# deepinv/deepinv

Measured on NVIDIA H100. Metric: pnp_pgd_iterations_per_s, higher is better.
Workload: dtype f32 (3 x FP16 split-operand tensor-core GEMMs: 22-bit operands, fp32 accumulate) + f32 operators

## Files before the change

### deepinv_b200/csrc/conv_tc32.cu

```cuda
#include "common.cuh"
#ifndef DINVK_EMUL
#include "tc_ptx.cuh"
#include "tma_tile.cuh"
#include <cuda_fp16.h>
#else
namespace dinvk { namespace tc {
inline void ldg256(const void* p, uint32_t (&r)[8]) { std::memcpy(r, p, 32); }
inline void stg256(void* p, const uint32_t (&r)[8]) { std::memcpy(p, r, 32); }
} }
#endif

#include <algorithm>
#include <cstdlib>
#include <cstring>

namespace dinvk {
namespace t32 {

constexpr int TX = 16, TY = 8;
constexpr int A_TILE = 128 * 128;
constexpr int B_TILE = 128 * 128;
constexpr int STAGE = 2 * A_TILE + B_TILE;
constexpr int STAGES = 4;
constexpr int STG_WARP = 16 * 32;
constexpr int SMEM = STAGES * STAGE + 8 * STG_WARP * 4 + 1024;
constexpr int THREADS = 2 * 128 + 32;

__device__ __forceinline__ float rna_tf32(float x) {
#ifndef DINVK_EMUL
  uint32_t u;
  asm("cvt.rna.tf32.f32 %0, %1;" : "=r"(u) : "f"(x));
  return __uint_as_float(u);
#else
  return __uint_as_float((__float_as_uint(x) + 0x1000u) & 0xffffe000u);
#endif
}

struct FmtTF32 {
  using elem = float;
  static constexpr int CH = 16, EB = 4, ID = 0;
  static constexpr float CORR = 1.0f;
#ifndef DINVK_EMUL
  static constexpr CUtensorMapDataType TM = CU_TENSOR_MAP_DATA_TYPE_FLOAT32;
#endif
};
struct FmtF16 {
  using elem = __half;
  static constexpr int CH = 32, EB = 2, ID = 1;
  static constexpr float CORR = 4.8828125e-4f;
#ifndef DINVK_EMUL
  static constexpr CUtensorMapDataType TM = CU_TENSOR_MAP_DATA_TYPE_FLOAT16;
#endif
};

#ifndef DINVK_EMUL
template <class F>
__device__ __forceinline__ void mma(float* d, uint32_t a_lo, uint32_t a_hi, uint32_t b_lo, uint32_t b_hi, uint32_t accumulate) {
  if constexpr (F::ID == 0) tc::wgmma_tf32_n64(d, a_lo, a_hi, b_lo, b_hi, accumulate);
  else tc::wgmma_f16_n64(d, a_lo, a_hi, b_lo, b_hi, accumulate);
}
template <class F>
__device__ __forceinline__ void mma_block64(float* acc, uint32_t a, uint32_t a_hi, uint32_t b, uint32_t b_hi, uint32_t fresh) {
  mma<F>(acc, a, a_hi, b, b_hi, fresh);
  mma<F>(acc + 32, a, a_hi, b + 512, b_hi, fresh);
  mma<F>(acc, a + 2, a_hi, b + 2, b_hi, 1u);
  mma<F>(acc + 32, a + 2, a_hi, b + 514, b_hi, 1u);
  mma<F>(acc + 32, a + 4, a_hi, b, b_hi, 1u);
  mma<F>(acc + 32, a + 6, a_hi, b + 2, b_hi, 1u);
}
template <class F>
__device__ __forceinline__ void mma128(float* d, uint32_t a_lo, uint32_t a_hi, uint32_t b_lo, uint32_t b_hi, uint32_t accumulate) {
  if constexpr (F::ID == 0) tc::wgmma_tf32_n128(d, a_lo, a_hi, b_lo, b_hi, accumulate);
  else tc::wgmma_f16_n128(d, a_lo, a_hi, b_lo, b_hi, accumulate);
}
template <class F>
__device__ __forceinline__ void mma_block128(float* acc, uint32_t w, uint32_t w_hi, uint32_t x, uint32_t x_hi, uint32_t fresh) {
  mma128<F>(acc, w, w_hi, x, x_hi, fresh);
  mma128<F>(acc + 64, w + 512, w_hi, x, x_hi, fresh);
  mma128<F>(acc, w + 2, w_hi, x + 2, x_hi, 1u);
  mma128<F>(acc + 64, w + 514, w_hi, x + 2, x_hi, 1u);
  mma128<F>(acc + 64, w, w_hi, x + 4, x_hi, 1u);
  mma128<F>(acc + 64, w + 2, w_hi, x + 6, x_hi, 1u);
}
template <class F, int N>
__device__ __forceinline__ void drain(float* v, const float* acc) {
#pragma unroll
  for (int i = 0; i < N / 2; ++i) v[i] += acc[i] + acc[N / 2 + i] * F::CORR;
}

__device__ __forceinline__ void release_stage(uint64_t* bar) {
  __syncwarp();
  if ((threadIdx.x & 31) == 0) tc::mbar_arrive(bar);
}

struct Maps {
  CUtensorMap a[4];
  CUtensorMap b;
};

struct Params {
  int B, H, W, Cin, Cout;
  int ntaps, kc_per_tap;
  int dx[9], dy[9], amap[9];
  int mode;
  int tiles_x, tiles_y, n_tiles;
  int relu;
  int win;
  const void* res;
  const void* res2;
  void* out;
  int* flag;
  const float* bias;
  int ngrp;
};

__device__ __forceinline__ void tile_index(const Params& P, int pixel_tiles, int t, int& pt, int& nt) {
  const int u = t / P.ngrp, lo = t - u * P.ngrp;
  const int hi = u / pixel_tiles;
  pt = u - hi * pixel_tiles;
  nt = hi * P.ngrp + lo;
}

#endif
template <class F>
__device__ __forceinline__ bool store_split(typename F::elem* p, const float* v) {
  uint32_t u[4][8];
  bool bad = false;
  if constexpr (F::ID == 0) {
#pragma unroll
    for (int i = 0; i < 16; ++i) {
      const float hi = rna_tf32(v[i]);
      u[i >> 3][i & 7] = __float_as_uint(hi);
      u[2 + (i >> 3)][i & 7] = __float_as_uint(v[i] - hi);
    }
  } else {
#pragma unroll
    for (int i = 0; i < 32; i += 2) {
      const __half h0 = __float2half_rn(v[i]), h1 = __float2half_rn(v[i + 1]);
      const __half l0 = __float2half_rn((v[i] - __half2float(h0)) * 2048.0f), l1 = __float2half_rn((v[i + 1] - __half2float(h1)) * 2048.0f);
      bad |= !(fabsf(v[i]) < 65000.0f) || !(fabsf(v[i + 1]) < 65000.0f);
      u[i >> 4][(i >> 1) & 7] = (uint32_t)__half_as_ushort(h0) | ((uint32_t)__half_as_ushort(h1) << 16);
      u[2 + (i >> 4)][(i >> 1) & 7] = (uint32_t)__half_as_ushort(l0) | ((uint32_t)__half_as_ushort(l1) << 16);
    }
  }
  char* pc = reinterpret_cast<char*>(p);
#pragma unroll
  for (int k = 0; k < 4; ++k) tc::stg256(pc + 32 * k, u[k]);
  return bad;
}
template <class F>
__device__ __forceinline__ void add_split_raw(const uint32_t (*raw)[8], float* v) {
  if constexpr (F::ID == 0) {
#pragma unroll
    for (int e = 0; e < 8; ++e) {
      v[e] += __uint_as_float(raw[0][e]) + __uint_as_float(raw[2][e]);
      v[8 + e] += __uint_as_float(raw[1][e]) + __uint_as_float(raw[3][e]);
    }
  } else {
#pragma unroll
    for (int c = 0; c < 2; ++c)
#pragma unroll
      for (int e = 0; e < 8; ++e) {
        const float2 h = __half22float2(*reinterpret_cast<const __half2*>(&raw[c][e]));
        const float2 l = __half22float2(*reinterpret_cast<const __half2*>(&raw[2 + c][e]));
        v[c * 16 + 2 * e] += h.x + l.x * F::CORR;
        v[c * 16 + 2 * e + 1] += h.y + l.y * F::CORR;
      }
  }
}
template <class F>
__device__ __forceinline__ void add_split(const typename F::elem* p, float* v) {
  uint32_t raw[4][8];
  const char* pc = reinterpret_cast<const char*>(p);
#pragma unroll
  for (int k = 0; k < 4; ++k) tc::ldg256(pc + 32 * k, raw[k]);
  add_split_raw<F>(raw, v);
}

#ifndef DINVK_EMUL
template <class F>
// ... 167 lines not shown
  __shared__ __align__(8) uint64_t full_bar[STAGES];
  __shared__ __align__(8) uint64_t empty_bar[STAGES];

  const int warp = threadIdx.x >> 5, lane = threadIdx.x & 31;
  const int pixel_tiles = P.B * P.tiles_y * P.tiles_x;
  const int total_tiles = pixel_tiles * P.n_tiles;
  const int nk = P.ntaps * P.kc_per_tap;

  if (threadIdx.x == 0) {
    tc::prefetch_tmap(&M.a[0]);
    tc::prefetch_tmap(&M.b);
    for (int s = 0; s < STAGES; ++s) { tc::mbar_init(&full_bar[s], 1); tc::mbar_init(&empty_bar[s], 8); }
    tc::fence_barrier_init();
  }
  __syncthreads();

  if (warp == 8) {
    if (lane == 0) {
      int s = 0; uint32_t ph = 0;
      for (int t = blockIdx.x; t < total_tiles; t += gridDim.x) {
        int pt, nt; tile_index(P, pixel_tiles, t, pt, nt);
        const int b = pt / (P.tiles_y * P.tiles_x), r = pt - b * (P.tiles_y * P.tiles_x);
        const int y0 = (r / P.tiles_x) * TY, x0 = (r % P.tiles_x) * TX;
        for (int kb = 0; kb < nk; ++kb) {
          const int tap = kb / P.kc_per_tap, kc = kb - tap * P.kc_per_tap;
          tc::mbar_wait(&empty_bar[s], ph ^ 1);
          uint8_t* sa = smem + s * STAGE;
          tc::mbar_arrive_expect_tx(&full_bar[s], STAGE);
          tc::tma_load_4d(sa, &M.a[P.amap[tap]], &full_bar[s], (2 * kc) * (2 * F::CH), x0 + P.dx[tap], y0 + P.dy[tap], b);
          tc::tma_load_4d(sa + A_TILE, &M.a[P.amap[tap]], &full_bar[s], (2 * kc + 1) * (2 * F::CH), x0 + P.dx[tap], y0 + P.dy[tap], b);
          tc::tma_load_2d(sa + 2 * A_TILE, &M.b, &full_bar[s], tap * P.Cin + kc * (2 * F::CH), nt * 128);
          if (++s == STAGES) { s = 0; ph ^= 1; }
        }
      }
    }
  } else {
    const int wg = warp >> 2;
    constexpr uint32_t HI = tc::desc_hi_sw128(1024);
    const uint32_t smem_lo = tc::smem_u32(smem) >> 4;
    int s = 0; uint32_t ph = 0;
    for (int t = blockIdx.x; t < total_tiles; t += gridDim.x) {
      int pt, nt; tile_index(P, pixel_tiles, t, pt, nt);
      const int b = pt / (P.tiles_y * P.tiles_x), r = pt - b * (P.tiles_y * P.tiles_x);
      const int y0 = (r / P.tiles_x) * TY, x0 = (r % P.tiles_x) * TX;
      float acc[64], v[32];
#pragma unroll
      for (int i = 0; i < 64; ++i) acc[i] = 0.f;
#pragma unroll
      for (int i = 0; i < 32; ++i) v[i] = 0.f;
      int in_win = 0;
      for (int kb = 0; kb < nk; ++kb) {
        tc::mbar_wait(&full_bar[s], ph);
        const uint32_t a0 = smem_lo + static_cast<uint32_t>(s) * (STAGE >> 4) + static_cast<uint32_t>(wg * (64 * 128 >> 4));
        const uint32_t b0 = smem_lo + static_cast<uint32_t>(s) * (STAGE >> 4) + (2 * A_TILE >> 4);
        tc::wgmma_fence();
#pragma unroll
        for (int jj = 0; jj < 2; ++jj)
          mma_block64<F>(acc, a0 + jj * (A_TILE >> 4), HI, b0 + jj * 4, HI, (jj | in_win) != 0 ? 1u : 0u);
        tc::wgmma_commit();
        tc::wgmma_wait<0>();
        tc::reg_fence<64>(acc);
        release_stage(&empty_bar[s]);
        if (++in_win == P.win || kb == nk - 1) {
          drain<F, 64>(v, acc);
          in_win = 0;
        }
        if (++s == STAGES) { s = 0; ph ^= 1; }
      }
      const int tap = P.mode == 2 ? nt * 64 / P.Cout : 0;
      const auto pixel_of = [&](int m) -> long long {
        const int mm = 64 * wg + 16 * (warp & 3) + m;
        const int y = y0 + mm / TX, x = x0 + mm % TX;
        if (!(y < P.H && x < P.W)) return -1;
        if (P.mode == 2) return ((long long)b * (2 * P.H) + 2 * y + (tap >> 1)) * (2LL * P.W) + 2 * x + (tap & 1);
        return ((long long)b * P.H + y) * P.W + x;
      };
      epilogue<F>(P, v, reinterpret_cast<float*>(smem + STAGES * STAGE) + warp * STG_WARP, pixel_of, nt * 64 - tap * P.Cout);
    }
  }
}

namespace slab {
constexpr int TXP = 16, TYP = 16;
constexpr int SLAB_X = TXP + 8, SLAB_Y = TYP + 2;
constexpr int SLAB_BYTES = SLAB_X * SLAB_Y * 128;
constexpr int A_STAGES = 2, B_STAGES = 6;
constexpr int WT_TILE = 128 * 128;
constexpr int CONSUMER_WARPS = 8;
constexpr int SMEM_BYTES = A_STAGES * SLAB_BYTES + B_STAGES * WT_TILE + CONSUMER_WARPS * STG_WARP * 4 + 1024;
constexpr int THREADS = 32 * CONSUMER_WARPS + 128;
constexpr int PRODUCER_REGS = 40, CONSUMER_REGS = 232;
static_assert(SLAB_BYTES % 1024 == 0, "slab stages must stay 1024-byte aligned");
static_assert(SMEM_BYTES <= 227 * 1024, "shared memory budget");
}

template <class F>
__global__ void __launch_bounds__(slab::THREADS, 1) conv_tc32_slab_kernel(const __grid_constant__ Maps M, const Params P) {
  using namespace slab;
  extern __shared__ uint8_t smem_raw[];
  uint8_t* smem = reinterpret_cast<uint8_t*>((reinterpret_cast<uintptr_t>(smem_raw) + 1023) & ~static_cast<uintptr_t>(1023));
  uint8_t* smem_b = smem + A_STAGES * SLAB_BYTES;
  __shared__ __align__(8) uint64_t afull[A_STAGES];
  __shared__ __align__(8) uint64_t aempty[A_STAGES];
  __shared__ __align__(8) uint64_t bfull[B_STAGES];
  __shared__ __align__(8) uint64_t bempty[B_STAGES];

  const int warp = threadIdx.x >> 5, lane = threadIdx.x & 31;
  const int pixel_tiles = P.B * P.tiles_y * P.tiles_x;
  const int total_tiles = pixel_tiles * P.n_tiles;
  const int nblk = P.Cin / F::CH;

  if (threadIdx.x == 0) {
    tc::prefetch_tmap(&M.a[0]);
    tc::prefetch_tmap(&M.b);
    for (int s = 0; s < A_STAGES; ++s) { tc::mbar_init(&afull[s], 1); tc::mbar_init(&aempty[s], CONSUMER_WARPS); }
    for (int s = 0; s < B_STAGES; ++s) { tc::mbar_init(&bfull[s], 1); tc::mbar_init(&bempty[s], CONSUMER_WARPS); }
    tc::fence_barrier_init();
  }
  __syncthreads();

  if (warp >= CONSUMER_WARPS) {
    tc::setmaxnreg_dec<PRODUCER_REGS>();
    if (warp == CONSUMER_WARPS && lane == 0) {
      int sa = 0; uint32_t pha = 0;
      int sb = 0; uint32_t phb = 0;
      for (int t = blockIdx.x; t < total_tiles; t += gridDim.x) {
        int pt, nt; tile_index(P, pixel_tiles, t, pt, nt);
        const int b = pt / (P.tiles_y * P.tiles_x), r = pt - b * (P.tiles_y * P.tiles_x);
        const int y0 = (r / P.tiles_x) * TYP, x0 = (r % P.tiles_x) * TXP;
        for (int j = 0; j < nblk; ++j) {
          tc::mbar_wait(&aempty[sa], pha ^ 1);
          tc::mbar_arrive_expect_tx(&afull[sa], SLAB_BYTES);
          tc::tma_load_4d(smem + sa * SLAB_BYTES, &M.a[0], &afull[sa], j * (2 * F::CH), x0 - 1, y0 - 1, b);
          if (++sa == A_STAGES) { sa = 0; pha ^= 1; }
          for (int tp = 0; tp < 5; ++tp) {
            tc::mbar_wait(&bempty[sb], phb ^ 1);
            tc::mbar_arrive_expect_tx(&bfull[sb], WT_TILE);
            tc::tma_load_2d(smem_b + sb * WT_TILE, &M.b, &bfull[sb], (j * 5 + tp) * (2 * F::CH), nt * 128);
            if (++sb == B_STAGES) { sb = 0; phb ^= 1; }
          }
        }
      }
    }
  } else {
    tc::setmaxnreg_inc<CONSUMER_REGS>();
    const int wg = warp >> 2;
    constexpr uint32_t HI_X = tc::desc_hi_sw128(SLAB_X * 128);
    constexpr uint32_t HI_W = tc::desc_hi_sw128(1024);
    const uint32_t slab_lo0 = (tc::smem_u32(smem) >> 4) + static_cast<uint32_t>(wg * 8 * 8);
    const uint32_t bt_lo0 = tc::smem_u32(smem_b) >> 4;
    int sa = 0; uint32_t pha = 0;
    int sb = 0; uint32_t phb = 0;
    for (int t = blockIdx.x; t < total_tiles; t += gridDim.x) {
      int pt, nt; tile_index(P, pixel_tiles, t, pt, nt);
      const int b = pt / (P.tiles_y * P.tiles_x), r = pt - b * (P.tiles_y * P.tiles_x);
      const int y0 = (r / P.tiles_x) * TYP, x0 = (r % P.tiles_x) * TXP;
      float acc[128], v[64];
#pragma unroll
      for (int i = 0; i < 128; ++i) acc[i] = 0.f;
#pragma unroll
      for (int i = 0; i < 64; ++i) v[i] = 0.f;
      int in_win = 0;
      int pend_b = -1;
      for (int j = 0; j < nblk; ++j) {
        tc::mbar_wait(&afull[sa], pha);
        const uint32_t slab_lo = slab_lo0 + static_cast<uint32_t>(sa) * (SLAB_BYTES >> 4);
        const uint32_t fresh = in_win == 0 ? 0u : 1u;
        const bool last_of_win = (in_win + 1 == P.win) || (j == nblk - 1);
#pragma unroll
        for (int tp = 0; tp < 5; ++tp) {
          tc::mbar_wait(&bfull[sb], phb);
          const uint32_t b_lo = bt_lo0 + static_cast<uint32_t>(sb) * (WT_TILE >> 4);
          tc::wgmma_fence();
#pragma unroll
          for (int par = 0; par < 2; ++par) {
            const int tap = 2 * tp + par;
            if (tap < 9) {
              const uint32_t x_t = slab_lo + static_cast<uint32_t>((tap / 3) * SLAB_X + (tap % 3)) * 8;
              mma_block128<F>(acc, b_lo + par * 4, HI_W, x_t, HI_X, tap == 0 ? fresh : 1u);
            }
          }
          tc::wgmma_commit();
          if (tp == 4) {
            tc::wgmma_wait<0>();
            tc::reg_fence<128>(acc);
            if (pend_b >= 0) release_stage(&bempty[pend_b]);
            release_stage(&bempty[sb]);
            release_stage(&aempty[sa]);
            pend_b = -1;
            if (last_of_win) drain<F, 128>(v, acc);
          } else {
            tc::wgmma_wait<1>();
            if (pend_b >= 0) release_stage(&bempty[pend_b]);
            pend_b = sb;
          }
          if (++sb == B_STAGES) { sb = 0; phb ^= 1; }
        }
        if (++sa == A_STAGES) { sa = 0; pha ^= 1; }
        in_win = last_of_win ? 0 : in_win + 1;
      }
      const auto pixel_of = [&](int n) -> long long {
        const int y = y0 + (n >> 3), x = x0 + 8 * wg + (n & 7);
        return y < P.H && x < P.W ? ((long long)b * P.H + y) * P.W + x : -1;
      };
      epilogue_t<F>(P, v, reinterpret_cast<float*>(smem_b + B_STAGES * WT_TILE) + warp * STG_WARP, pixel_of, nt * 64 + 16 * (warp & 3));
    }
  }
}

#endif
struct HeadParams {
  const float* x; const float* w; const float* bias; void* out;
  int B, C, H, W, Cout;
  float fill_scalar; const float* fill_batch; int has_fill; int relu;
  int* flag;
};

template <class F, int CT>
__global__ void __launch_bounds__(256) head_tc32_kernel(const HeadParams P) {
  constexpr int KR = 9 * CT, KP = (KR + 3) & ~3;
#ifndef DINVK_EMUL
  extern __shared__ __align__(16) float sw[];
#else
  float* sw = reinterpret_cast<float*>(::emul::dyn_smem());
#endif
  for (int i = threadIdx.x; i < P.Cout * KP; i += blockDim.x) {
    const int co = i / KP, k = i - co * KP;
    sw[i] = k < KR ? __ldg(P.w + co * KR + k) : 0.f;
  }
  __syncthreads();
  const long long npix = (long long)P.B * P.H * P.W;
  const long long p = (long long)blockIdx.x * blockDim.x + threadIdx.x;
  if (p >= npix) return;
  const long long HW = (long long)P.H * P.W;
  const int b = (int)(p / HW);
  const int rem = (int)(p - (long long)b * HW);
  const int y = rem / P.W, x = rem - y * P.W;
  const float fillv = P.has_fill ? (P.fill_batch ? __ldg(P.fill_batch + b) : P.fill_scalar) : 0.f;
  float in[KP];
#pragma unroll
  for (int k = KR; k < KP; ++k) in[k] = 0.f;
  const float* img = P.x + (long long)b * P.C * HW;
#pragma unroll
  for (int c = 0; c < CT; ++c) {
#pragma unroll
    for (int tap = 0; tap < 9; ++tap) {
      const int yy = y + tap / 3 - 1, xx = x + tap % 3 - 1;
      const bool inb = (yy >= 0) && (yy < P.H) && (xx >= 0) && (xx < P.W);
      float val = 0.f;
      if (inb) val = (c < P.C) ? __ldg(img + (long long)c * HW + (long long)yy * P.W + xx) : fillv;
      in[c * 9 + tap] = val;
    }
  }
  typename F::elem* o = static_cast<typename F::elem*>(P.out) + p * P.Cout * 2;
  bool bad = false;
  for (int c0 = 0; c0 < P.Cout; c0 += F::CH) {
    float v[F::CH];
#pragma unroll
    for (int i = 0; i < F::CH; ++i) {
      float a = P.bias ? __ldg(P.bias + c0 + i) : 0.f;
      const float4* wr = reinterpret_cast<const float4*>(sw + (c0 + i) * KP);
#pragma unroll
      for (int k = 0; k < KP / 4; ++k) {
// ... 375 lines not shown
}

static int default_window() {
  static int w = -1;
  if (w < 0) {
    const char* e = getenv("DINVK_TC32_WINDOW");
    w = e ? std::max(1, atoi(e)) : 4;
  }
  return w;
}

template <class F>
static int conv_generic(const void* x, const void* weight, const float* bias, const void* res, const void* res2, void* out, int B, int H,
                        int W, int Cin, int Cout, int kind, int act, int window, int* flag, void* stream) {
  DINVK_CHECK_ARG(x && weight && out, "conv_tc32: null pointer");
  DINVK_CHECK_ARG(B >= 0 && H >= 1 && W >= 1, "conv_tc32: bad shape");
  DINVK_CHECK_ARG(kind >= 0 && kind <= 2, "conv_tc32: kind=%d not in 0..2", kind);
  DINVK_CHECK_ARG(Cin % (2 * F::CH) == 0 && Cin >= 2 * F::CH, "conv_tc32: Cin=%d must be a multiple of %d", Cin, 2 * F::CH);
  DINVK_CHECK_ARG(Cout % 64 == 0 && Cout >= 64, "conv_tc32: Cout=%d must be a multiple of 64", Cout);
  DINVK_CHECK_ARG(kind != 1 || (H % 2 == 0 && W % 2 == 0), "conv_tc32: 2x2 stride-2 needs even H, W");
  DINVK_CHECK_ARG(kind == 0 || (!res && !res2), "conv_tc32: residual inputs are for kind 0 only");
  DINVK_CHECK_ARG(epilogue_aligned(bias, res, res2, out), "conv_tc32: bias, res, res2 and out must be 16-byte aligned");
  if (B == 0) return DINVK_OK;
  Maps M;
  Params P{};
  int rc;
  const uint64_t px = (uint64_t)Cin * 2 * F::EB;
  P.B = B; P.Cin = Cin; P.Cout = Cout;
  P.kc_per_tap = Cin / (2 * F::CH);
  P.relu = act; P.res = res; P.res2 = res2; P.out = out; P.bias = bias; P.flag = flag;
  P.win = window > 0 ? window : default_window();
  const uint32_t abox[4] = {2 * F::CH, TX, TY, 1};
  long long K = Cin, rows = 2LL * Cout;
  if (kind == 1) {
    const int Ho = H / 2, Wo = W / 2;
    const uint64_t adims[4] = {(uint64_t)Cin * 2, (uint64_t)Wo, (uint64_t)Ho, (uint64_t)B}, astrides[3] = {2 * px, 2 * px * W, px * W * H};
    for (int t = 0; t < 4; ++t) {
      const char* base = reinterpret_cast<const char*>(x) + ((long long)(t >> 1) * W + (t & 1)) * px;
      if ((rc = map_split<F>(&M.a[t], base, 4, adims, astrides, abox, "tc32 activations"))) return rc;
      P.amap[t] = t;
    }
    K = 4LL * Cin;
    P.H = Ho; P.W = Wo; P.ntaps = 4; P.n_tiles = Cout / 64;
  } else {
    const uint64_t adims[4] = {(uint64_t)Cin * 2, (uint64_t)W, (uint64_t)H, (uint64_t)B}, astrides[3] = {px, px * W, px * W * H};
    if ((rc = map_split<F>(&M.a[0], x, 4, adims, astrides, abox, "tc32 activations"))) return rc;
    M.a[1] = M.a[0]; M.a[2] = M.a[0]; M.a[3] = M.a[0];
    P.H = H; P.W = W;
    if (kind == 0) {
      K = 9LL * Cin;
      P.ntaps = 9; P.n_tiles = Cout / 64;
      for (int t = 0; t < 9; ++t) { P.dx[t] = t % 3 - 1; P.dy[t] = t / 3 - 1; }
    } else {
      rows = 8LL * Cout;
      P.ntaps = 1; P.mode = 2; P.n_tiles = 4 * Cout / 64;
    }
  }
  const uint64_t wdims[2] = {(uint64_t)K, (uint64_t)rows}, wstride = (uint64_t)K * F::EB;
  const uint32_t wbox[2] = {2 * F::CH, 128};
  if ((rc = map_split<F>(&M.b, weight, 2, wdims, &wstride, wbox, "tc32 weights"))) return rc;
  P.tiles_x = ceil_div(P.W, TX); P.tiles_y = ceil_div(P.H, TY);
  P.ngrp = getenv("DINVK_TC32_NT_OUTER") ? 1 : P.n_tiles;
  return launch_persistent(conv_tc32_kernel<F>, THREADS, SMEM, (long long)P.B * P.tiles_y * P.tiles_x * P.n_tiles, stream, M, P);
}

template <class F>
static int conv_slab(const void* x, const void* weight, const float* bias, const void* res, const void* res2, void* out, int B, int H, int W,
                     int Cin, int Cout, int act, int window, int* flag, void* stream) {
  DINVK_CHECK_ARG(x && weight && out, "conv_tc32_slab: null pointer");
  DINVK_CHECK_ARG(B >= 0 && H >= 1 && W >= 1, "conv_tc32_slab: bad shape");
  DINVK_CHECK_ARG(Cin % F::CH == 0 && Cin >= F::CH, "conv_tc32_slab: Cin=%d must be a multiple of %d", Cin, F::CH);
  DINVK_CHECK_ARG(Cout % 64 == 0 && Cout >= 64, "conv_tc32_slab: Cout=%d must be a multiple of 64", Cout);
  DINVK_CHECK_ARG(epilogue_aligned(bias, res, res2, out), "conv_tc32_slab: bias, res, res2 and out must be 16-byte aligned");
  if (B == 0) return DINVK_OK;
  Maps M;
  Params P{};
  int rc;
  const uint64_t px = (uint64_t)Cin * 2 * F::EB;
  const uint64_t adims[4] = {(uint64_t)Cin * 2, (uint64_t)W, (uint64_t)H, (uint64_t)B}, astrides[3] = {px, px * W, px * W * H};
  const uint32_t abox[4] = {2 * F::CH, slab::SLAB_X, slab::SLAB_Y, 1};
  if ((rc = map_split<F>(&M.a[0], x, 4, adims, astrides, abox, "tc32 activations"))) return rc;
  M.a[1] = M.a[0]; M.a[2] = M.a[0]; M.a[3] = M.a[0];
  const uint64_t wdims[2] = {10ull * Cin, 2ull * Cout}, wstride = 10ull * Cin * F::EB;
  const uint32_t wbox[2] = {2 * F::CH, 128};
  if ((rc = map_split<F>(&M.b, weight, 2, wdims, &wstride, wbox, "tc32 weights"))) return rc;
  P.B = B; P.H = H; P.W = W; P.Cin = Cin; P.Cout = Cout;
  P.ntaps = 9; P.kc_per_tap = Cin / F::CH; P.n_tiles = Cout / 64;
  for (int t = 0; t < 9; ++t) { P.dx[t] = t % 3 - 1; P.dy[t] = t / 3 - 1; }
  P.relu = act; P.res = res; P.res2 = res2; P.out = out; P.bias = bias; P.flag = flag;
  static const int def_win = getenv("DINVK_TC32_SLAB_WINDOW") ? std::max(1, atoi(getenv("DINVK_TC32_SLAB_WINDOW"))) : 1;
  P.win = window > 0 ? window : def_win;
  P.tiles_x = ceil_div(W, slab::TXP); P.tiles_y = ceil_div(H, slab::TYP);
  {
    static const int env_g = getenv("DINVK_TC32_NT_GROUP") ? atoi(getenv("DINVK_TC32_NT_GROUP")) : 0;
    int g = env_g > 0 ? env_g : 2;
    while (g > 1 && P.n_tiles % g) --g;
    P.ngrp = std::max(1, std::min(g, P.n_tiles));
  }
  return launch_persistent(conv_tc32_slab_kernel<F>, slab::THREADS, slab::SMEM_BYTES, (long long)P.B * P.tiles_y * P.tiles_x * P.n_tiles,
                           stream, M, P);
}

#endif
template <class F>
static int conv_head(const float* x_nchw, const float* weight, const float* bias, void* out, int B, int C, int H, int W, int Cout,
                     float fill_scalar, const float* fill_batch, int has_fill, int act, int* flag, void* stream) {
  const int CT = C + (has_fill ? 1 : 0);
  DINVK_CHECK_ARG(Cout % F::CH == 0 && Cout >= F::CH && Cout <= 256, "conv_tc32_head: Cout=%d must be a multiple of %d (<= 256)", Cout, F::CH);
  HeadParams P{x_nchw, weight, bias, out, B, C, H, W, Cout, fill_scalar, fill_batch, has_fill, act, flag};
  const long long npix = (long long)B * H * W;
  static const bool old_head = getenv("DINVK_TC32_OLD_HEAD") != nullptr;
  if (Cout == 64 && CT >= 1 && CT <= 4 && !old_head) {
    const long long warps = (long long)B * ceil_div(H, 2) * ceil_div(W, 32);
    const unsigned g = (unsigned)((warps + 7) / 8);
    switch (CT) {
      case 1: DINVK_LAUNCH((head64_tc32_kernel<F, 1>), dim3(g), dim3(256), 0, stream, P); break;
      case 2: DINVK_LAUNCH((head64_tc32_kernel<F, 2>), dim3(g), dim3(256), 0, stream, P); break;
      case 3: DINVK_LAUNCH((head64_tc32_kernel<F, 3>), dim3(g), dim3(256), 0, stream, P); break;
      default: DINVK_LAUNCH((head64_tc32_kernel<F, 4>), dim3(g), dim3(256), 0, stream, P); break;
    }
    return DINVK_POST_LAUNCH();
  }
  const unsigned grid = (unsigned)((npix + 255) / 256);
  const size_t smem = (size_t)Cout * ((9 * CT + 3) & ~3) * 4;
  switch (CT) {
    case 1: DINVK_LAUNCH((head_tc32_kernel<F, 1>), dim3(grid), dim3(256), smem, stream, P); break;
    case 2: DINVK_LAUNCH((head_tc32_kernel<F, 2>), dim3(grid), dim3(256), smem, stream, P); break;
    case 3: DINVK_LAUNCH((head_tc32_kernel<F, 3>), dim3(grid), dim3(256), smem, stream, P); break;
    default: DINVK_LAUNCH((head_tc32_kernel<F, 4>), dim3(grid), dim3(256), smem, stream, P); break;
  }
  return DINVK_POST_LAUNCH();
}

template <class F>
static int conv_tail(const void* x, const float* weight, const float* bias, const float* add_nchw, float* out_nchw, int B, int H, int W,
                     int Cin, int Cout, const int* flag, void* stream) {
  DINVK_CHECK_ARG(Cin % F::CH == 0 && Cin >= F::CH && Cin <= 128, "conv_tc32_tail: Cin=%d must be a multiple of %d (<= 128)", Cin, F::CH);
  TailParams P{x, weight, bias, add_nchw, out_nchw, B, H, W, Cin, Cout, flag};
  static const bool old_tail = getenv("DINVK_TC32_OLD_TAIL") != nullptr;
  if (Cin == 64 && Cout >= 1 && Cout <= 4 && !old_tail) {
    const int co = Cout == 3 ? 4 : Cout, wt = 16 / co;
    const long long warps = (long long)B * ceil_div(W, wt) * ceil_div(H, TL_RC);
    const unsigned grid = (unsigned)((warps + 7) / 8);
    if (co == 1) DINVK_LAUNCH((tail64_tc32_kernel<F, 1>), dim3(grid), dim3(256), 0, stream, P);
    else if (co == 2) DINVK_LAUNCH((tail64_tc32_kernel<F, 2>), dim3(grid), dim3(256), 0, stream, P);
    else DINVK_LAUNCH((tail64_tc32_kernel<F, 4>), dim3(grid), dim3(256), 0, stream, P);
    return DINVK_POST_LAUNCH();
  }
  const int tiles = B * ceil_div(H, TL_TY) * ceil_div(W, TL_TX);
  const int CO = Cout <= 2 ? 2 : 4;
  const size_t smem = ((size_t)(TL_TY + 2) * (TL_TX + 2) * (Cin + 4) + (size_t)CO * 9 * Cin) * 4;
  int rc;
  if (CO == 2) {
    if ((rc = allow_smem(tail_tc32_kernel<F, 2>, smem))) return rc;
    DINVK_LAUNCH((tail_tc32_kernel<F, 2>), dim3(tiles), dim3(256), smem, stream, P);
  } else {
    if ((rc = allow_smem(tail_tc32_kernel<F, 4>, smem))) return rc;
    DINVK_LAUNCH((tail_tc32_kernel<F, 4>), dim3(tiles), dim3(256), smem, stream, P);
  }
  return DINVK_POST_LAUNCH();
}

}
}

using namespace dinvk;

#define DINVK_FMT_DISPATCH(fmt, call_tf32, call_f16)                                                   \
// ... 68 lines not shown
```

### deepinv_b200/csrc/tc_ptx.cuh

```cuda
#pragma once
#include <cstdint>
#include <cuda.h>
#include <cuda_bf16.h>
#include <cuda_runtime.h>

namespace dinvk {
namespace tc {

__device__ __forceinline__ uint32_t smem_u32(const void* p) { return static_cast<uint32_t>(__cvta_generic_to_shared(p)); }

__device__ __forceinline__ bool elect_one() {
  uint32_t pred = 0;
  asm volatile(
      "{\n\t"
      ".reg .pred P;\n\t"
      "elect.sync _|P, 0xffffffff;\n\t"
      "selp.u32 %0, 1, 0, P;\n\t"
      "}\n"
      : "=r"(pred));
  return pred != 0;
}

__device__ __forceinline__ void mbar_init(uint64_t* bar, uint32_t count) {
  asm volatile("mbarrier.init.shared::cta.b64 [%0], %1;" ::"r"(smem_u32(bar)), "r"(count));
}
__device__ __forceinline__ void fence_barrier_init() { asm volatile("fence.mbarrier_init.release.cluster;" ::: "memory"); }
__device__ __forceinline__ void fence_proxy_async() { asm volatile("fence.proxy.async.shared::cta;" ::: "memory"); }
__device__ __forceinline__ void mbar_arrive_expect_tx(uint64_t* bar, uint32_t bytes) {
  asm volatile("mbarrier.arrive.expect_tx.shared::cta.b64 _, [%0], %1;" ::"r"(smem_u32(bar)), "r"(bytes) : "memory");
}
__device__ __forceinline__ void mbar_arrive(uint64_t* bar) {
  asm volatile("mbarrier.arrive.shared::cta.b64 _, [%0];" ::"r"(smem_u32(bar)) : "memory");
}
__device__ __forceinline__ bool mbar_try_wait(uint64_t* bar, uint32_t parity) {
  uint32_t ok;
  asm volatile(
      "{\n\t"
      ".reg .pred P;\n\t"
      "mbarrier.try_wait.parity.shared::cta.b64 P, [%1], %2;\n\t"
      "selp.u32 %0, 1, 0, P;\n\t"
      "}\n"
      : "=r"(ok)
      : "r"(smem_u32(bar)), "r"(parity)
      : "memory");
  return ok != 0;
}
__device__ __forceinline__ void mbar_wait(uint64_t* bar, uint32_t parity) {
  while (!mbar_try_wait(bar, parity)) {
  }
}

__device__ __forceinline__ void prefetch_tmap(const CUtensorMap* m) {
  asm volatile("prefetch.tensormap [%0];" ::"l"(reinterpret_cast<uint64_t>(m)) : "memory");
}
__device__ __forceinline__ void tma_load_2d(void* smem, const CUtensorMap* m, uint64_t* bar, int c0, int c1) {
  asm volatile("cp.async.bulk.tensor.2d.shared::cluster.global.mbarrier::complete_tx::bytes [%0], [%1, {%3, %4}], [%2];" ::"r"(
                   smem_u32(smem)),
               "l"(reinterpret_cast<uint64_t>(m)), "r"(smem_u32(bar)), "r"(c0), "r"(c1)
               : "memory");
}
__device__ __forceinline__ void tma_load_4d(void* smem, const CUtensorMap* m, uint64_t* bar, int c0, int c1, int c2, int c3) {
  asm volatile(
      "cp.async.bulk.tensor.4d.shared::cluster.global.mbarrier::complete_tx::bytes [%0], [%1, {%3, %4, %5, %6}], [%2];" ::"r"(
          smem_u32(smem)),
      "l"(reinterpret_cast<uint64_t>(m)), "r"(smem_u32(bar)), "r"(c0), "r"(c1), "r"(c2), "r"(c3)
      : "memory");
}

__device__ __forceinline__ void wgmma_fence() { asm volatile("wgmma.fence.sync.aligned;" ::: "memory"); }
__device__ __forceinline__ void wgmma_commit() { asm volatile("wgmma.commit_group.sync.aligned;" ::: "memory"); }
template <int N>
__device__ __forceinline__ void wgmma_wait() { asm volatile("wgmma.wait_group.sync.aligned %0;" ::"n"(N) : "memory"); }
template <int N>
__device__ __forceinline__ void reg_fence(float* d) {
#pragma unroll
  for (int i = 0; i < N; ++i) asm volatile("" : "+f"(d[i])::"memory");
}

template <uint32_t N>
__device__ __forceinline__ void setmaxnreg_dec() { asm volatile("setmaxnreg.dec.sync.aligned.u32 %0;" ::"n"(N)); }
template <uint32_t N>
__device__ __forceinline__ void setmaxnreg_inc() { asm volatile("setmaxnreg.inc.sync.aligned.u32 %0;" ::"n"(N)); }

__host__ __device__ constexpr uint32_t desc_hi_sw128(uint32_t sbo_bytes) { return ((sbo_bytes >> 4) & 0x3FFF) | (1u << 30); }

__device__ __forceinline__ void wgmma_bf16_n16(float* d, uint32_t a_lo, uint32_t a_hi, uint32_t b_lo, uint32_t b_hi, uint32_t scale_d) {
  asm volatile(
      "{\n\t.reg .pred p;\n\t.reg .b64 da, db;\n\t"
      "mov.b64 da, {%8, %9};\n\tmov.b64 db, {%10, %11};\n\tsetp.ne.b32 p, %12, 0;\n\t"
      "wgmma.mma_async.sync.aligned.m64n16k16.f32.bf16.bf16 {%0, %1, %2, %3, %4, %5, %6, %7}, da, db, p, 1, 1, 0, 0;\n\t}\n"
      : "+f"(d[0]), "+f"(d[1]), "+f"(d[2]), "+f"(d[3]), "+f"(d[4]), "+f"(d[5]), "+f"(d[6]), "+f"(d[7])
      : "r"(a_lo | (1u << 16)), "r"(a_hi), "r"(b_lo | (1u << 16)), "r"(b_hi), "r"(scale_d)
      : "memory");
}
__device__ __forceinline__ void wgmma_bf16_n64(float* d, uint32_t a_lo, uint32_t a_hi, uint32_t b_lo, uint32_t b_hi, uint32_t scale_d) {
  asm volatile(
      "{\n\t.reg .pred p;\n\t.reg .b64 da, db;\n\t"
      "mov.b64 da, {%32, %33};\n\tmov.b64 db, {%34, %35};\n\tsetp.ne.b32 p, %36, 0;\n\t"
      "wgmma.mma_async.sync.aligned.m64n64k16.f32.bf16.bf16 {%0, %1, %2, %3, %4, %5, %6, %7, %8, %9, %10, %11, %12, %13, %14, %15, %16, %17, %18, %19, %20, %21, %22, %23, %24, %25, %26, %27, %28, %29, %30, %31}, da, db, p, 1, 1, 0, 0;\n\t}\n"
      : "+f"(d[0]), "+f"(d[1]), "+f"(d[2]), "+f"(d[3]), "+f"(d[4]), "+f"(d[5]), "+f"(d[6]), "+f"(d[7]),
        "+f"(d[8]), "+f"(d[9]), "+f"(d[10]), "+f"(d[11]), "+f"(d[12]), "+f"(d[13]), "+f"(d[14]), "+f"(d[15]),
        "+f"(d[16]), "+f"(d[17]), "+f"(d[18]), "+f"(d[19]), "+f"(d[20]), "+f"(d[21]), "+f"(d[22]), "+f"(d[23]),
        "+f"(d[24]), "+f"(d[25]), "+f"(d[26]), "+f"(d[27]), "+f"(d[28]), "+f"(d[29]), "+f"(d[30]), "+f"(d[31])
      : "r"(a_lo | (1u << 16)), "r"(a_hi), "r"(b_lo | (1u << 16)), "r"(b_hi), "r"(scale_d)
      : "memory");
}
__device__ __forceinline__ void wgmma_bf16_n128(float* d, uint32_t a_lo, uint32_t a_hi, uint32_t b_lo, uint32_t b_hi, uint32_t scale_d) {
  asm volatile(
      "{\n\t.reg .pred p;\n\t.reg .b64 da, db;\n\t"
      "mov.b64 da, {%64, %65};\n\tmov.b64 db, {%66, %67};\n\tsetp.ne.b32 p, %68, 0;\n\t"
      "wgmma.mma_async.sync.aligned.m64n128k16.f32.bf16.bf16 {%0, %1, %2, %3, %4, %5, %6, %7, %8, %9, %10, %11, %12, %13, %14, %15, %16, %17, %18, %19, %20, %21, %22, %23, %24, %25, %26, %27, %28, %29, %30, %31, %32, %33, %34, %35, %36, %37, %38, %39, %40, %41, %42, %43, %44, %45, %46, %47, %48, %49, %50, %51, %52, %53, %54, %55, %56, %57, %58, %59, %60, %61, %62, %63}, da, db, p, 1, 1, 0, 0;\n\t}\n"
      : "+f"(d[0]), "+f"(d[1]), "+f"(d[2]), "+f"(d[3]), "+f"(d[4]), "+f"(d[5]), "+f"(d[6]), "+f"(d[7]),
        "+f"(d[8]), "+f"(d[9]), "+f"(d[10]), "+f"(d[11]), "+f"(d[12]), "+f"(d[13]), "+f"(d[14]), "+f"(d[15]),
        "+f"(d[16]), "+f"(d[17]), "+f"(d[18]), "+f"(d[19]), "+f"(d[20]), "+f"(d[21]), "+f"(d[22]), "+f"(d[23]),
        "+f"(d[24]), "+f"(d[25]), "+f"(d[26]), "+f"(d[27]), "+f"(d[28]), "+f"(d[29]), "+f"(d[30]), "+f"(d[31]),
        "+f"(d[32]), "+f"(d[33]), "+f"(d[34]), "+f"(d[35]), "+f"(d[36]), "+f"(d[37]), "+f"(d[38]), "+f"(d[39]),
        "+f"(d[40]), "+f"(d[41]), "+f"(d[42]), "+f"(d[43]), "+f"(d[44]), "+f"(d[45]), "+f"(d[46]), "+f"(d[47]),
        "+f"(d[48]), "+f"(d[49]), "+f"(d[50]), "+f"(d[51]), "+f"(d[52]), "+f"(d[53]), "+f"(d[54]), "+f"(d[55]),
        "+f"(d[56]), "+f"(d[57]), "+f"(d[58]), "+f"(d[59]), "+f"(d[60]), "+f"(d[61]), "+f"(d[62]), "+f"(d[63])
      : "r"(a_lo | (1u << 16)), "r"(a_hi), "r"(b_lo | (1u << 16)), "r"(b_hi), "r"(scale_d)
      : "memory");
}
__device__ __forceinline__ void wgmma_f16_n64(float* d, uint32_t a_lo, uint32_t a_hi, uint32_t b_lo, uint32_t b_hi, uint32_t scale_d) {
  asm volatile(
      "{\n\t.reg .pred p;\n\t.reg .b64 da, db;\n\t"
      "mov.b64 da, {%32, %33};\n\tmov.b64 db, {%34, %35};\n\tsetp.ne.b32 p, %36, 0;\n\t"
      "wgmma.mma_async.sync.aligned.m64n64k16.f32.f16.f16 {%0, %1, %2, %3, %4, %5, %6, %7, %8, %9, %10, %11, %12, %13, %14, %15, %16, %17, %18, %19, %20, %21, %22, %23, %24, %25, %26, %27, %28, %29, %30, %31}, da, db, p, 1, 1, 0, 0;\n\t}\n"
      : "+f"(d[0]), "+f"(d[1]), "+f"(d[2]), "+f"(d[3]), "+f"(d[4]), "+f"(d[5]), "+f"(d[6]), "+f"(d[7]),
        "+f"(d[8]), "+f"(d[9]), "+f"(d[10]), "+f"(d[11]), "+f"(d[12]), "+f"(d[13]), "+f"(d[14]), "+f"(d[15]),
        "+f"(d[16]), "+f"(d[17]), "+f"(d[18]), "+f"(d[19]), "+f"(d[20]), "+f"(d[21]), "+f"(d[22]), "+f"(d[23]),
        "+f"(d[24]), "+f"(d[25]), "+f"(d[26]), "+f"(d[27]), "+f"(d[28]), "+f"(d[29]), "+f"(d[30]), "+f"(d[31])
      : "r"(a_lo | (1u << 16)), "r"(a_hi), "r"(b_lo | (1u << 16)), "r"(b_hi), "r"(scale_d)
      : "memory");
}
__device__ __forceinline__ void wgmma_tf32_n64(float* d, uint32_t a_lo, uint32_t a_hi, uint32_t b_lo, uint32_t b_hi, uint32_t scale_d) {
  asm volatile(
      "{\n\t.reg .pred p;\n\t.reg .b64 da, db;\n\t"
      "mov.b64 da, {%32, %33};\n\tmov.b64 db, {%34, %35};\n\tsetp.ne.b32 p, %36, 0;\n\t"
      "wgmma.mma_async.sync.aligned.m64n64k8.f32.tf32.tf32 {%0, %1, %2, %3, %4, %5, %6, %7, %8, %9, %10, %11, %12, %13, %14, %15, %16, %17, %18, %19, %20, %21, %22, %23, %24, %25, %26, %27, %28, %29, %30, %31}, da, db, p, 1, 1;\n\t}\n"
      : "+f"(d[0]), "+f"(d[1]), "+f"(d[2]), "+f"(d[3]), "+f"(d[4]), "+f"(d[5]), "+f"(d[6]), "+f"(d[7]),
        "+f"(d[8]), "+f"(d[9]), "+f"(d[10]), "+f"(d[11]), "+f"(d[12]), "+f"(d[13]), "+f"(d[14]), "+f"(d[15]),
        "+f"(d[16]), "+f"(d[17]), "+f"(d[18]), "+f"(d[19]), "+f"(d[20]), "+f"(d[21]), "+f"(d[22]), "+f"(d[23]),
        "+f"(d[24]), "+f"(d[25]), "+f"(d[26]), "+f"(d[27]), "+f"(d[28]), "+f"(d[29]), "+f"(d[30]), "+f"(d[31])
      : "r"(a_lo | (1u << 16)), "r"(a_hi), "r"(b_lo | (1u << 16)), "r"(b_hi), "r"(scale_d)
      : "memory");
}

__device__ __forceinline__ void wgmma_f16_n128(float* d, uint32_t a_lo, uint32_t a_hi, uint32_t b_lo, uint32_t b_hi, uint32_t scale_d) {
  asm volatile(
      "{\n\t.reg .pred p;\n\t.reg .b64 da, db;\n\t"
      "mov.b64 da, {%64, %65};\n\tmov.b64 db, {%66, %67};\n\tsetp.ne.b32 p, %68, 0;\n\t"
      "wgmma.mma_async.sync.aligned.m64n128k16.f32.f16.f16 {%0, %1, %2, %3, %4, %5, %6, %7, %8, %9, %10, %11, %12, %13, %14, %15, %16, %17, %18, %19, %20, %21, %22, %23, %24, %25, %26, %27, %28, %29, %30, %31, %32, %33, %34, %35, %36, %37, %38, %39, %40, %41, %42, %43, %44, %45, %46, %47, %48, %49, %50, %51, %52, %53, %54, %55, %56, %57, %58, %59, %60, %61, %62, %63}, da, db, p, 1, 1, 0, 0;\n\t}\n"
      : "+f"(d[0]), "+f"(d[1]), "+f"(d[2]), "+f"(d[3]), "+f"(d[4]), "+f"(d[5]), "+f"(d[6]), "+f"(d[7]),
        "+f"(d[8]), "+f"(d[9]), "+f"(d[10]), "+f"(d[11]), "+f"(d[12]), "+f"(d[13]), "+f"(d[14]), "+f"(d[15]),
        "+f"(d[16]), "+f"(d[17]), "+f"(d[18]), "+f"(d[19]), "+f"(d[20]), "+f"(d[21]), "+f"(d[22]), "+f"(d[23]),
        "+f"(d[24]), "+f"(d[25]), "+f"(d[26]), "+f"(d[27]), "+f"(d[28]), "+f"(d[29]), "+f"(d[30]), "+f"(d[31]),
        "+f"(d[32]), "+f"(d[33]), "+f"(d[34]), "+f"(d[35]), "+f"(d[36]), "+f"(d[37]), "+f"(d[38]), "+f"(d[39]),
        "+f"(d[40]), "+f"(d[41]), "+f"(d[42]), "+f"(d[43]), "+f"(d[44]), "+f"(d[45]), "+f"(d[46]), "+f"(d[47]),
        "+f"(d[48]), "+f"(d[49]), "+f"(d[50]), "+f"(d[51]), "+f"(d[52]), "+f"(d[53]), "+f"(d[54]), "+f"(d[55]),
        "+f"(d[56]), "+f"(d[57]), "+f"(d[58]), "+f"(d[59]), "+f"(d[60]), "+f"(d[61]), "+f"(d[62]), "+f"(d[63])
      : "r"(a_lo | (1u << 16)), "r"(a_hi), "r"(b_lo | (1u << 16)), "r"(b_hi), "r"(scale_d)
      : "memory");
}
__device__ __forceinline__ void wgmma_tf32_n128(float* d, uint32_t a_lo, uint32_t a_hi, uint32_t b_lo, uint32_t b_hi, uint32_t scale_d) {
  asm volatile(
      "{\n\t.reg .pred p;\n\t.reg .b64 da, db;\n\t"
      "mov.b64 da, {%64, %65};\n\tmov.b64 db, {%66, %67};\n\tsetp.ne.b32 p, %68, 0;\n\t"
// ... 25 lines not shown
```

Measured before the change: 10.38.

## Shrink slab halo and load only half-width weight tile for tap 8

Cuts the activation slab width from TXP+8 to TXP+2 columns, which removes unused halo pixels from each TMA load, and pads each slab stage to 1024-byte alignment. The padded 10th weight slot (tap 9 of the paired layout) is no longer fetched: a separate 64B-swizzled tensor map loads only the tap-8 half tile, and the final wgmma block uses the matching descriptor and offset. The shared memory this frees goes to a seventh weight stage. The approach depends on correct SW64 descriptor encoding, and the x-slab stride no longer being a multiple of 1024 could break swizzle-atom assumptions.

```diff
diff --git a/deepinv_b200/csrc/conv_tc32.cu b/deepinv_b200/csrc/conv_tc32.cu
--- a/deepinv_b200/csrc/conv_tc32.cu
+++ b/deepinv_b200/csrc/conv_tc32.cu
@@ -73,12 +73,12 @@
   if constexpr (F::ID == 0) tc::wgmma_tf32_n128(d, a_lo, a_hi, b_lo, b_hi, accumulate);
   else tc::wgmma_f16_n128(d, a_lo, a_hi, b_lo, b_hi, accumulate);
 }
-template <class F>
+template <class F, uint32_t LO = 512>
 __device__ __forceinline__ void mma_block128(float* acc, uint32_t w, uint32_t w_hi, uint32_t x, uint32_t x_hi, uint32_t fresh) {
   mma128<F>(acc, w, w_hi, x, x_hi, fresh);
-  mma128<F>(acc + 64, w + 512, w_hi, x, x_hi, fresh);
+  mma128<F>(acc + 64, w + LO, w_hi, x, x_hi, fresh);
   mma128<F>(acc, w + 2, w_hi, x + 2, x_hi, 1u);
-  mma128<F>(acc + 64, w + 514, w_hi, x + 2, x_hi, 1u);
+  mma128<F>(acc + 64, w + LO + 2, w_hi, x + 2, x_hi, 1u);
   mma128<F>(acc + 64, w, w_hi, x + 4, x_hi, 1u);
   mma128<F>(acc + 64, w + 2, w_hi, x + 6, x_hi, 1u);
 }
@@ -96,6 +96,7 @@
 struct Maps {
   CUtensorMap a[4];
   CUtensorMap b;
+  CUtensorMap b8;
 };
 
 struct Params {
@@ -429,15 +430,16 @@
 
 namespace slab {
 constexpr int TXP = 16, TYP = 16;
-constexpr int SLAB_X = TXP + 8, SLAB_Y = TYP + 2;
+constexpr int SLAB_X = TXP + 2, SLAB_Y = TYP + 2;
 constexpr int SLAB_BYTES = SLAB_X * SLAB_Y * 128;
-constexpr int A_STAGES = 2, B_STAGES = 6;
+constexpr int SLAB_STAGE = (SLAB_BYTES + 1023) / 1024 * 1024;
+constexpr int A_STAGES = 2, B_STAGES = 7;
 constexpr int WT_TILE = 128 * 128;
+constexpr int T8_TILE = 128 * 64;
 constexpr int CONSUMER_WARPS = 8;
-constexpr int SMEM_BYTES = A_STAGES * SLAB_BYTES + B_STAGES * WT_TILE + CONSUMER_WARPS * STG_WARP * 4 + 1024;
+constexpr int SMEM_BYTES = A_STAGES * SLAB_STAGE + B_STAGES * WT_TILE + CONSUMER_WARPS * STG_WARP * 4 + 1024;
 constexpr int THREADS = 32 * CONSUMER_WARPS + 128;
 constexpr int PRODUCER_REGS = 40, CONSUMER_REGS = 232;
-static_assert(SLAB_BYTES % 1024 == 0, "slab stages must stay 1024-byte aligned");
 static_assert(SMEM_BYTES <= 227 * 1024, "shared memory budget");
 }
 
@@ -446,7 +448,7 @@
   using namespace slab;
   extern __shared__ uint8_t smem_raw[];
   uint8_t* smem = reinterpret_cast<uint8_t*>((reinterpret_cast<uintptr_t>(smem_raw) + 1023) & ~static_cast<uintptr_t>(1023));
-  uint8_t* smem_b = smem + A_STAGES * SLAB_BYTES;
+  uint8_t* smem_b = smem + A_STAGES * SLAB_STAGE;
   __shared__ __align__(8) uint64_t afull[A_STAGES];
   __shared__ __align__(8) uint64_t aempty[A_STAGES];
   __shared__ __align__(8) uint64_t bfull[B_STAGES];
@@ -460,6 +462,7 @@
   if (threadIdx.x == 0) {
     tc::prefetch_tmap(&M.a[0]);
     tc::prefetch_tmap(&M.b);
+    tc::prefetch_tmap(&M.b8);
     for (int s = 0; s < A_STAGES; ++s) { tc::mbar_init(&afull[s], 1); tc::mbar_init(&aempty[s], CONSUMER_WARPS); }
     for (int s = 0; s < B_STAGES; ++s) { tc::mbar_init(&bfull[s], 1); tc::mbar_init(&bempty[s], CONSUMER_WARPS); }
     tc::fence_barrier_init();
@@ -478,12 +481,12 @@
         for (int j = 0; j < nblk; ++j) {
           tc::mbar_wait(&aempty[sa], pha ^ 1);
           tc::mbar_arrive_expect_tx(&afull[sa], SLAB_BYTES);
-          tc::tma_load_4d(smem + sa * SLAB_BYTES, &M.a[0], &afull[sa], j * (2 * F::CH), x0 - 1, y0 - 1, b);
+          tc::tma_load_4d(smem + sa * SLAB_STAGE, &M.a[0], &afull[sa], j * (2 * F::CH), x0 - 1, y0 - 1, b);
           if (++sa == A_STAGES) { sa = 0; pha ^= 1; }
           for (int tp = 0; tp < 5; ++tp) {
             tc::mbar_wait(&bempty[sb], phb ^ 1);
-            tc::mbar_arrive_expect_tx(&bfull[sb], WT_TILE);
-            tc::tma_load_2d(smem_b + sb * WT_TILE, &M.b, &bfull[sb], (j * 5 + tp) * (2 * F::CH), nt * 128);
+            tc::mbar_arrive_expect_tx(&bfull[sb], tp < 4 ? WT_TILE : T8_TILE);
+            tc::tma_load_2d(smem_b + sb * WT_TILE, tp < 4 ? &M.b : &M.b8, &bfull[sb], (j * 5 + tp) * (2 * F::CH), nt * 128);
             if (++sb == B_STAGES) { sb = 0; phb ^= 1; }
           }
         }
@@ -494,6 +497,7 @@
     const int wg = warp >> 2;
     constexpr uint32_t HI_X = tc::desc_hi_sw128(SLAB_X * 128);
     constexpr uint32_t HI_W = tc::desc_hi_sw128(1024);
+    constexpr uint32_t HI_W8 = tc::desc_hi_sw64(512);
     const uint32_t slab_lo0 = (tc::smem_u32(smem) >> 4) + static_cast<uint32_t>(wg * 8 * 8);
     const uint32_t bt_lo0 = tc::smem_u32(smem_b) >> 4;
     int sa = 0; uint32_t pha = 0;
@@ -511,7 +515,7 @@
       int pend_b = -1;
       for (int j = 0; j < nblk; ++j) {
         tc::mbar_wait(&afull[sa], pha);
-        const uint32_t slab_lo = slab_lo0 + static_cast<uint32_t>(sa) * (SLAB_BYTES >> 4);
+        const uint32_t slab_lo = slab_lo0 + static_cast<uint32_t>(sa) * (SLAB_STAGE >> 4);
         const uint32_t fresh = in_win == 0 ? 0u : 1u;
         const bool last_of_win = (in_win + 1 == P.win) || (j == nblk - 1);
 #pragma unroll
@@ -522,10 +526,11 @@
 #pragma unroll
           for (int par = 0; par < 2; ++par) {
             const int tap = 2 * tp + par;
-            if (tap < 9) {
-              const uint32_t x_t = slab_lo + static_cast<uint32_t>((tap / 3) * SLAB_X + (tap % 3)) * 8;
+            const uint32_t x_t = slab_lo + static_cast<uint32_t>((tap / 3) * SLAB_X + (tap % 3)) * 8;
+            if (tap < 8)
               mma_block128<F>(acc, b_lo + par * 4, HI_W, x_t, HI_X, tap == 0 ? fresh : 1u);
-            }
+            else if (tap == 8)
+              mma_block128<F, 256>(acc, b_lo, HI_W8, x_t, HI_X, 1u);
           }
           tc::wgmma_commit();
           if (tp == 4) {
@@ -1067,8 +1072,11 @@
   if ((rc = map_split<F>(&M.a[0], x, 4, adims, astrides, abox, "tc32 activations"))) return rc;
   M.a[1] = M.a[0]; M.a[2] = M.a[0]; M.a[3] = M.a[0];
   const uint64_t wdims[2] = {10ull * Cin, 2ull * Cout}, wstride = 10ull * Cin * F::EB;
-  const uint32_t wbox[2] = {2 * F::CH, 128};
+  const uint32_t wbox[2] = {2 * F::CH, 128}, w8box[2] = {F::CH, 128};
   if ((rc = map_split<F>(&M.b, weight, 2, wdims, &wstride, wbox, "tc32 weights"))) return rc;
+  if ((rc = encode_tiled(&M.b8, F::TM, 2, weight, wdims, &wstride, w8box, CU_TENSOR_MAP_SWIZZLE_64B, CU_TENSOR_MAP_L2_PROMOTION_L2_256B,
+                         "tc32 weights (tap 8)")))
+    return rc;
   P.B = B; P.H = H; P.W = W; P.Cin = Cin; P.Cout = Cout;
   P.ntaps = 9; P.kc_per_tap = Cin / F::CH; P.n_tiles = Cout / 64;
   for (int t = 0; t < 9; ++t) { P.dx[t] = t % 3 - 1; P.dy[t] = t / 3 - 1; }
diff --git a/deepinv_b200/csrc/tc_ptx.cuh b/deepinv_b200/csrc/tc_ptx.cuh
--- a/deepinv_b200/csrc/tc_ptx.cuh
+++ b/deepinv_b200/csrc/tc_ptx.cuh
@@ -83,6 +83,7 @@
 __device__ __forceinline__ void setmaxnreg_inc() { asm volatile("setmaxnreg.inc.sync.aligned.u32 %0;" ::"n"(N)); }
 
 __host__ __device__ constexpr uint32_t desc_hi_sw128(uint32_t sbo_bytes) { return ((sbo_bytes >> 4) & 0x3FFF) | (1u << 30); }
+__host__ __device__ constexpr uint32_t desc_hi_sw64(uint32_t sbo_bytes) { return ((sbo_bytes >> 4) & 0x3FFF) | (2u << 30); }
 
 __device__ __forceinline__ void wgmma_bf16_n16(float* d, uint32_t a_lo, uint32_t a_hi, uint32_t b_lo, uint32_t b_hi, uint32_t scale_d) {
   asm volatile(
```

Result: no change. 10.47 (median of 6 runs) (+0.9%).
